# chenglou/ai-font-renderer

Hardware: AMD Instinct MI355X
Metric: glyphs/sec training (batch fwd+bwd+step) (higher is better)
Workload: dtype bf16; 1 GPU; C3: 32x32 glyph MLP 32->1024->1024->1024, char+font embedding, batch 8192/GPU (BASELINE configs[2]; per-GPU shard of configs[3]); per_gpu_batch=8192, global_batch=8192, parallelism=single, params=2137152

## Files before the change

### ai-font-renderer_amd/csrc/afr_api.hip

```cpp
#include "afr_common.h"
#include "../../include/afr.h"
static_assert(AFR_LOSS_MSE == LOSS_MSE && AFR_LOSS_BCE == LOSS_BCE, "afr.h and afr_common.h name the same loss kinds");

#include <cmath>
#include <cstdarg>
#include <cstdio>
#include <cstring>
#include <map>
#include <string>
#include <utility>
#include <vector>

static thread_local char g_err[512] = "";
static int fail(int code, const char* fmt, ...) {
    va_list ap;
    va_start(ap, fmt);
    vsnprintf(g_err, sizeof g_err, fmt, ap);
    va_end(ap);
    return code;
}
#define HIPCHK(expr)                                                                          \
    do {                                                                                      \
        hipError_t e_ = (expr);                                                               \
        if (e_ != hipSuccess) return fail(AFR_EHIP, "%s: %s", #expr, hipGetErrorString(e_)); \
// ... 39 lines not shown
    char* ws = nullptr;
    size_t ws_bytes = 0, ws_need = 0;
    int device = -1;
    bool defer = false;
    int pend_tile256 = 0;
    std::vector<GemmParams> pend;
    std::vector<std::string> pend_tag;
    double pend_flops = 0.0, pend_bytes = 0.0;
    unsigned* pend_arrived = nullptr;
    size_t o_shadow = 0, o_err = 0, o_loss = 0, o_u = 0, o_z = 0, o_dz = 0, o_slab_e = 0, o_save = 0;
    std::vector<size_t> o_act;
    size_t o_d[2] = {0, 0};
    size_t o_table = 0;
    size_t o_dw1 = 0;
    int k0 = 0;
    bool fused1 = false;
    bool wT_valid = false;
    size_t o_w1t = 0, o_w2t = 0, o_slab1 = 0;
    bool l1f = false; size_t o_l1f = 0;
    bool combo_ok = false, combo_on = false; size_t o_h1c = 0, o_h0c = 0, o_cidx = 0; int h1c_ld = 0;
    std::vector<size_t> o_mbits; bool mbits_on = false;
    size_t o_shadow2 = 0; int shadow_cur = 0;
    bool step_on = false; AdamArgs st{};
    std::vector<int64_t> adam_done;
    struct PixBlock { int64_t ln1g, ln1b, win, bin, wo, bo, ln2g, ln2b, w1, b1, w2, b2; };
    std::vector<PixBlock> pix;
    int64_t px_pos = 0, px_emb = 0, px_font = -1, px_lnfg = 0, px_lnfb = 0, px_wout = 0, px_bout = 0;
    struct PixSave { size_t hin, h1, n1, q, o, n2, kv, f, ln1p, ln2p, fbits; };
    std::vector<PixSave> pxs;
    size_t o_ctx = 0, o_a = 0, o_hf = 0, o_dh = 0, o_dht = 0, o_df = 0, o_dn = 0, o_dq = 0, o_dkvp = 0, o_dkv = 0, o_dkvt = 0, o_dctxt = 0,
           o_dctx = 0, o_headp = 0;
    struct Layer { int N, K; int64_t w_off, b_off; int sk = 1; size_t o_slab_w = 0, o_slab_b = 0;
                   size_t o_cnt = 0; int n_cnt = 0; unsigned coop_arrived = 0; };
    std::vector<Layer> layers;
    std::vector<Layer> pxl;
    int64_t emb_off = 0, font_off = 0;
    int64_t s_pos = 0, s_emb = 0, s_win = 0, s_bin = 0, s_wo = 0, s_bo = 0, s_g = 0, s_b = 0, s_w1 = 0, s_b1 = 0, s_wout = 0, s_bout = 0;
    const int64_t* last_x = nullptr;
    const int64_t* last_font = nullptr;
    int last_B = 0, last_L = 0, last_ldx = 0, last_training = 0;
    uint64_t last_step = 0;
    bool have_du = false;
    bool have_u = false;
    int next_stage = 0;
    const int64_t* ds_x = nullptr; const int64_t* ds_font = nullptr; const void* ds_target = nullptr;
    int ds_tdtype = 0, ds_L = 0; int64_t ds_rows = 0;
// ... 875 lines not shown
            h = p->ws + p->o_h1c;
            first = 1;
        } else if (p->k0) {
            const auto& l = p->layers[0];
            ProfScope ps(p, s, "glyph_l1_fwd", 0.0, (double)B * l.N * p->act_bytes);
            HIPCHK(afr_launch_glyph_l1_fwd(c.dtype, p->P + p->emb_off, femb, p->P + l.w_off, p->P + l.b_off, x, font, B, c.embed_dim,
                                           l.N, c.vocab, c.n_fonts, (float*)(p->ws + p->o_table), h, p->ws + p->o_act[1], err, s,
                                           p->l1f ? (void*)(p->ws + p->o_w1t) : nullptr));
            h = p->ws + p->o_act[1];
            first = 1;
        } else {
            ProfScope ps(p, s, "glyph_embed", 0.0, 0.0);
            HIPCHK(afr_launch_glyph_embed(c.dtype, p->P + p->emb_off, femb, x, font, B, c.embed_dim, c.vocab, c.n_fonts, h, err, s));
        }
        const bool bits = fl != nullptr && c.dtype == AFR_BF16;
        for (int i = first; i < nl; ++i) {
            const auto& l = p->layers[i];
            const bool last = (i == nl - 1);
            void* outp = last ? u : (void*)(p->ws + p->o_act[i + 1]);
            GemmParams g = lin_fwd(p, l, h, outp, B, last ? 0 : AFR_GEMM_RELU);
            if (combo && i == 1) { g.a_rowmap = (const int*)(p->ws + p->o_cidx); g.lda = p->h1c_ld; }
            if (bits && !last && p->o_mbits[i]) { g.mask_out = (unsigned char*)(p->ws + p->o_mbits[i]); g.ldmask = l.N / 8; }
            if (last && fl) g.loss = *fl;
            int rc = run_gemm(p, s, g);
            if (rc) return rc;
            h = outp;
        }
        p->last_L = 1;
    }
    if (y) {
        ProfScope ps(p, s, c.loss == AFR_LOSS_BCE ? "sigmoid_out" : "clamp_out", 0.0, 0.0);
        HIPCHK(afr_launch_clamp_out(c.dtype, u, y, (long long)B * Pix, s, c.loss));
    }
    p->last_x = x; p->last_font = font; p->last_B = B; p->last_training = training; p->last_step = step;
    p->next_stage = 0;
    p->combo_on = c.kind == AFR_KIND_GLYPH && fl != nullptr && p->k0 && combo_for(p, B);
    p->mbits_on = c.kind == AFR_KIND_GLYPH && fl != nullptr && c.dtype == AFR_BF16;
    p->have_du = fl != nullptr;
    p->have_u = fl == nullptr;
    return AFR_OK;
}
extern "C" int afr_forward(afr_plan* p, const int64_t* x, const int64_t* font, int B, int L, float* y, int training,
                           uint64_t step, void* stream) {
    return forward_impl(p, x, font, B, L, y, training, step, stream, nullptr);
}

// ... 159 lines not shown
            return AFR_OK;
        }
        if ((rc = run_gemm(p, s, lin_dx(p, p->layers[0], du, p->ws + p->o_dz, nullptr, B)))) return rc;
        if ((rc = sheet_front_bwd(p, s, rt, 7.0e6))) return rc;
        if ((rc = flush())) return rc;
        if (g_off) *g_off = 0;
        if (g_len) *g_len = p->s_wout;
        return AFR_OK;
    }
    const int nl = (int)p->layers.size();
    const int i = nl - 1 - stage;
    auto& l = p->layers[i];
    const void* a = p->ws + p->o_act[i];
    const void* dy = stage == 0 ? du : (const void*)(p->ws + p->o_d[(stage - 1) & 1]);
    if (i == 0 && p->k0) {
        const int K0 = p->k0, E = c.embed_dim;
        if (p->l1f && !(c.reserved & AFR_CFG_L1_BWD_UNFUSED)) {
            float* sl = (float*)(p->ws + p->o_l1f);
            const int CS = afr_glyph_l1_bwd_fused_split(B, l.N), nb = afr_glyph_l1_bwd_fused_blocks(B, l.N), nc = l.N / CS;
            const long long st = afr_glyph_l1_bwd_fused_slab_floats(B, l.N, c.vocab, c.n_fonts);
            {
                ProfScope ps(p, s, "glyph_l1_bwd_fused", 2.0 * B * l.N * (2.0 * E + 1.0), (double)B * l.N * 2.0 + (double)nb * st * 4.0);
                if (p->combo_on) HIPCHK(afr_launch_glyph_l1_bwd_fused(dy, l.N, p->ws + p->o_h0c, E, p->ws + p->o_w1t, p->last_x, p->last_font, B, l.N,
                                                                      c.vocab, c.n_fonts, sl, s, (const int*)(p->ws + p->o_cidx)));
                else HIPCHK(afr_launch_glyph_l1_bwd_fused(dy, l.N, a, K0, p->ws + p->o_w1t, p->last_x, p->last_font, B, l.N, c.vocab, c.n_fonts, sl, s));
            }
            for (int cs = 0; cs < CS; ++cs) {
                afr_rtable_add(rt, p->G + l.w_off + (size_t)cs * nc * E, sl + (size_t)cs * st, nb / CS, st * CS, (long long)nc * E);
                afr_rtable_add(rt, p->G + l.b_off + (size_t)cs * nc, sl + (size_t)cs * st + (size_t)nc * E, nb / CS, st * CS, nc);
            }
            afr_rtable_add(rt, p->G + p->emb_off, sl + (size_t)nc * E + nc, nb, st, (long long)c.vocab * E);
            if (c.n_fonts > 0) afr_rtable_add(rt, p->G + p->font_off, sl + (size_t)nc * E + nc + (size_t)c.vocab * E, nb, st, (long long)c.n_fonts * E);
            if ((rc = flush())) return rc;
            if (g_off) *g_off = 0;
            if (g_len) *g_len = l.b_off + (l.N + 63) / 64 * 64;
            return AFR_OK;
        }
        int sk = choose_splitk(l.N, K0, B);
        if (sk > l.sk) sk = l.sk;
        float* sw = (float*)(p->ws + l.o_slab_w);
        float* sb = (float*)(p->ws + l.o_slab_b);
        const long long stride = (long long)l.N * K0;
        if ((rc = run_gemm(p, s, lin_dw(dy, a, sw, sk == 1 ? p->G + l.b_off : sb, B, l.N, K0, sk, sk == 1 ? 0 : stride)))) return rc;
        if (sk > 1) afr_rtable_add(rt, p->G + l.b_off, sb, sk, l.N, l.N);
        float* dw1 = (float*)(p->ws + p->o_dw1);
        float* part = (float*)(p->ws + p->o_slab_e);
        {
            ProfScope ps(p, s, "glyph_l1_bwd", 0.0, (double)sk * l.N * K0 * 4.0);
// ... 390 lines not shown
                           int L, int64_t mean_elems, float* loss_accum, uint64_t step, int do_step, float lr, float b1,
                           float b2, float eps, float wd, int64_t t, void* stream) {
    int rc;
    if ((rc = check_loss_args(target, tdtype, mean_elems, loss_accum))) return rc;
    if (!p || !p->P) return fail(AFR_ESTATE, "plan has no bound parameters");
    if ((rc = ema_guard(p, "afr_train_step"))) return rc;
    DevGuard dg(p->device);
    const AdamArgs h{lr, b1, b2, eps, wd, t};
    const bool fuse_opt = do_step && !(p->cfg.reserved & AFR_CFG_UNFUSED_OPTIMIZER) && !(p->clip_norm > 0.f);
    if (p->fused1 && !(p->cfg.reserved & AFR_CFG_NO_FUSED_GLYPH1)) {
        if (!p->G) return fail(AFR_ESTATE, "plan has no bound gradient buffer");
        RTable rt;
        if ((rc = glyph1_fused(p, x, font, target, tdtype, rowmap, B, mean_elems, loss_accum, (hipStream_t)stream, rt))) return rc;
        if (fuse_opt && moments_bound(p)) {
            if (t < 1) return fail(AFR_EINVAL, "t starts at 1");
            rc = reduce_and_step(p, (hipStream_t)stream, rt, h);
            p->wT_valid = rc == AFR_OK;
            return rc;
        }
        if ((rc = run_reduce_group(p, (hipStream_t)stream, rt))) return rc;
        if (do_step && (rc = afr_adamw_step(p, lr, b1, b2, eps, wd, t, 1.f, stream))) return rc;
        return AFR_OK;
    }
    const LossArgs fl = loss_args(p, true, target, tdtype, rowmap, mean_elems, loss_accum);
    if ((rc = forward_impl(p, x, font, B, L, nullptr, 1, step, stream, &fl))) return rc;
    if (fuse_opt && fused_step_eligible(p, B)) {
        if (t < 1) return fail(AFR_EINVAL, "t starts at 1");
        return sheet_fused_step(p, (hipStream_t)stream, h);
    }
    if (fuse_opt && moments_bound(p) && p->cfg.kind != AFR_KIND_PIXEL) {
        if (t < 1) return fail(AFR_EINVAL, "t starts at 1");
        const int n = afr_backward_stages(p);
        RTable rt;
        p->step_on = true; p->adam_done.clear(); p->st = h;
        for (int st = 0; st < n; ++st)
            if ((rc = backward_stage_impl(p, st, nullptr, nullptr, (hipStream_t)stream, &rt))) { p->step_on = false; return rc; }
        p->step_on = false;
        p->next_stage = 0;
        p->have_du = false;
        return reduce_and_step(p, (hipStream_t)stream, rt, h);
    }
    if ((rc = afr_backward(p, stream))) return rc;
    if (do_step && (rc = afr_adamw_step(p, lr, b1, b2, eps, wd, t, 1.f, stream))) return rc;
    return AFR_OK;
}
extern "C" int afr_train_step(afr_plan* p, const int64_t* x, const int64_t* font, const void* target, int tdtype, int B,
                              int L, int64_t mean_elems, float* loss_accum, uint64_t step, int do_step, float lr, float b1,
                              float b2, float eps, float wd, int64_t t, void* stream) {
    return train_step_impl(p, x, font, target, tdtype, nullptr, B, L, mean_elems, loss_accum, step, do_step, lr, b1, b2, eps, wd, t, stream);
}

extern "C" int afr_bind_dataset(afr_plan* p, const int64_t* x, const int64_t* font, const void* target, int tdtype, int64_t n_rows, int L) {
    if (!p) return fail(AFR_EINVAL, "null plan");
    if (!x && !font && !target) {
        p->ds_x = p->ds_font = nullptr; p->ds_target = nullptr; p->ds_rows = 0; p->ds_L = 0;
        return AFR_OK;
    }
    if (n_rows >= (1ll << 31)) return fail(AFR_EUNSUPPORTED, "a data set of %lld rows: row indices are narrowed to 32 bits (fewer than 2^31 rows)", (long long)n_rows);
    if (!x || !target || n_rows <= 0) return fail(AFR_EINVAL, "a data set needs codes, targets and at least one row");
// ... 455 lines not shown
```

### ai-font-renderer_amd/csrc/afr_common.h

```cpp
#pragma once
#include <hip/hip_runtime.h>
#include <stdint.h>
#include <stddef.h>
#include <type_traits>

typedef __bf16 bf16_t;
typedef __attribute__((ext_vector_type(4))) float f32x4;
typedef __attribute__((ext_vector_type(16))) float f32x16;
typedef __attribute__((ext_vector_type(8))) __bf16 bf16x8;
typedef __attribute__((ext_vector_type(4))) __bf16 bf16x4;
typedef __attribute__((ext_vector_type(4))) short s16x4;

__host__ __device__ __forceinline__ uint32_t afr_hash32(uint64_t idx, uint32_t key) {
    uint32_t lo = (uint32_t)idx, hi = (uint32_t)(idx >> 32);
    uint32_t h = lo * 0x9E3779B1u + (key + hi * 0x85EBCA6Bu);
    h ^= h >> 16; h *= 0x21F0AAADu;
    h ^= h >> 15; h *= 0x735A2D97u;
    h ^= h >> 15;
    return h;
}
__host__ __device__ __forceinline__ bool afr_keep(uint64_t idx, uint32_t key, uint32_t thr24) {
    return (afr_hash32(idx, key) >> 8) < thr24;
}

// ... 1 lines not shown
    uint64_t z = x + 0x9E3779B97F4A7C15ull;
    z = (z ^ (z >> 30)) * 0xBF58476D1CE4E5B9ull;
    z = (z ^ (z >> 27)) * 0x94D049BB133111EBull;
    return z ^ (z >> 31);
}
enum { AFR_STREAM_EMBED = 1, AFR_STREAM_ATTN = 2, AFR_STREAM_FC = 3 };
static inline uint32_t afr_dropout_key(uint64_t seed, uint64_t step, uint64_t stream, uint64_t rank) {
    uint64_t v = seed ^ (step * 0x9E3779B97F4A7C15ull) ^ (stream * 0xC2B2AE3D27D4EB4Full) ^ (rank * 0x165667B19E3779F9ull);
    return (uint32_t)(afr_splitmix64(v) & 0xFFFFFFFFull);
}
static inline uint32_t afr_keep_threshold(float keep_prob) { return (uint32_t)((double)keep_prob * 16777216.0); }

__device__ __forceinline__ float wave_sum(float v) {
#pragma unroll
    for (int o = 32; o > 0; o >>= 1) v += __shfl_xor(v, o, 64);
    return v;
}
__device__ __forceinline__ float wave_max(float v) {
#pragma unroll
    for (int o = 32; o > 0; o >>= 1) v = fmaxf(v, __shfl_xor(v, o, 64));
    return v;
}

__device__ __forceinline__ void loss_block_finish(float block_sum, float* partial, unsigned* counter, float* loss_accum,
                                                  float inv_n, float* sh) {
    __shared__ unsigned ticket_;
    if (threadIdx.x == 0) {
        __hip_atomic_store(partial + blockIdx.x, block_sum, __ATOMIC_RELAXED, __HIP_MEMORY_SCOPE_AGENT);
        asm volatile("s_waitcnt vmcnt(0)" ::: "memory");
        ticket_ = __hip_atomic_fetch_add(counter, 1u, __ATOMIC_RELAXED, __HIP_MEMORY_SCOPE_AGENT);
    }
    __syncthreads();
    if (ticket_ != gridDim.x - 1) return;
    float a = 0.f;
    for (int i = threadIdx.x; i < (int)gridDim.x; i += blockDim.x)
        a += __hip_atomic_load(partial + i, __ATOMIC_RELAXED, __HIP_MEMORY_SCOPE_AGENT);
    sh[threadIdx.x] = a;
    __syncthreads();
    for (int o = blockDim.x >> 1; o > 0; o >>= 1) {
        if ((int)threadIdx.x < o) sh[threadIdx.x] += sh[threadIdx.x + o];
        __syncthreads();
    }
    if (threadIdx.x == 0) {
        loss_accum[0] += sh[0] * inv_n;
        __hip_atomic_store(counter, 0u, __ATOMIC_RELAXED, __HIP_MEMORY_SCOPE_AGENT);
    }
}

constexpr int LOSS_MSE = 0, LOSS_BCE = 1;
__device__ __forceinline__ float sigmoid_of(float u, float e) {
    const float r = __builtin_amdgcn_rcpf(1.f + e);
    return u >= 0.f ? r : e * r;
}
__device__ __forceinline__ float sigmoid_f(float u) { return sigmoid_of(u, __expf(-fabsf(u))); }
__device__ __forceinline__ float bce_logits_elem(float u, float t, float inv_n, float& du) {
    const float e = __expf(-fabsf(u));
    du = (sigmoid_of(u, e) - t) * inv_n;
    return fmaf(-t, u, fmaxf(u, 0.f)) + __logf(1.f + e);
}
template <int LOSS>
__device__ __forceinline__ float loss_elem(float u, float t, float inv_n, float g2, float& du) {
    if constexpr (LOSS == LOSS_BCE) return bce_logits_elem(u, t, inv_n, du);
    else {
        const float diff = fminf(fmaxf(u, 0.f), 1.f) - t;
        du = (u >= 0.f && u <= 1.f) ? g2 * diff : 0.f;
        return diff * diff;
    }
}
template <bool LUT>
// ... 73 lines not shown
    int M, N, K;
    int lda, ldb, ldc, ldaux;
    int flags;
    int splitk;
    long long slab_stride;
    float* colsum = nullptr;
    long long colsum_stride = 0;
    LossArgs loss;
    float* ad_p = nullptr; float* ad_m = nullptr; float* ad_v = nullptr; bf16_t* ad_shadow = nullptr;
    AdamHyper ad;
    int head_tiles = 0;
    int ad_kind = OPT_ADAMW;
    float* fix_ws = nullptr; unsigned* fix_cnt = nullptr;
    float* coop_ws = nullptr; unsigned* coop_cnt = nullptr; unsigned coop_target = 0; uint32_t* err = nullptr;
    const int* a_rowmap = nullptr; const int* b_rowmap = nullptr; const int* aux_rowmap = nullptr;
    float out_scale = 1.f;
    unsigned char* mask_out = nullptr; const unsigned char* mask_in = nullptr; int ldmask = 0;
#ifdef AFR_GEMM_TIMING
    int dbg_slot = 0;
#endif
};
constexpr uint32_t AFR_ERR_INDEX = 1u, AFR_ERR_COOP_TIMEOUT = 2u, AFR_ERR_ROW = 4u, AFR_ERR_GRAD_NONFINITE = 8u;
hipError_t afr_launch_gemm(int dtype, const GemmParams& p, hipStream_t s);
hipError_t afr_launch_gemm_fp8(const GemmParams& p, hipStream_t s);
hipError_t afr_launch_f32_to_fp8(const float* src, unsigned char* dst, long long n, float inv_scale, hipStream_t s);
bool afr_gemm_groupable(int dtype, const GemmParams& p);
hipError_t afr_launch_gemm_group(int dtype, const GemmParams* ps, int n, int tile256, hipStream_t s);
void afr_gemm_pair_plan(int B, int n_out, int k_in, int* tile256, int* splitk);
constexpr size_t AFR_FIX_SLICE_BYTES = 256 * 256 * 4;
hipError_t afr_launch_gemm_fix(const GemmParams& p, hipStream_t s);
const char* afr_gemm_kernel_name(int dtype, const GemmParams& p);
bool afr_gemm_wide_ok(int M, int N, int K);

hipError_t afr_launch_reduce(float* dst, const float* slabs, int nslabs, long long slab_stride, long long n,
                             float scale, int accumulate, hipStream_t s);
struct RSeg {
    float* dst; const float* src; long long stride; long long n4; int nslabs; int blk0; int nblk; int deep;
    bf16_t* shT = nullptr; int tN = 0, tK = 0;
};
constexpr int AFR_RT_MAXSEG = 32;
constexpr int AFR_L1F_MAX_SPLIT = 4;
struct RTable {
    int nseg = 0; int nblocks = 0; int overflow = 0;
    int adam = 0; AdamHyper ad;
    const float* gbase; float* P; float* M; float* V; bf16_t* shadow;
    RSeg seg[AFR_RT_MAXSEG];
// ... 35 lines not shown
                                   int* ridx, int64_t* sx, int64_t* sfont, uint32_t* err_flag, hipStream_t s);
hipError_t afr_launch_f32_to_bf16(const float* src, bf16_t* dst, long long n, hipStream_t s);
hipError_t afr_launch_clamp_bwd(int act_dtype, void* u_inout, const float* dy, long long n, hipStream_t s, int loss_kind = LOSS_MSE);
hipError_t afr_launch_clamp_out(int act_dtype, const void* u, float* y, long long n, hipStream_t s, int loss_kind = LOSS_MSE);
hipError_t afr_launch_glyph_embed(int act_dtype, const float* emb, const float* font_emb, const int64_t* x,
                                  const int64_t* font, int B, int E, int vocab, int n_fonts, void* out,
                                  uint32_t* err_flag, hipStream_t s);
int afr_embed_bwd_blocks(int B);
hipError_t afr_launch_glyph_l1_fwd(int act_dtype, const float* emb, const float* font_emb, const float* W1, const float* b1,
                                   const int64_t* x, const int64_t* font, int B, int E, int N1, int vocab, int n_fonts,
                                   float* table, void* h0, void* h1, uint32_t* err_flag, hipStream_t s, void* w1t = nullptr);
hipError_t afr_launch_glyph_combo(const float* emb, const float* font_emb, const float* W1, const float* b1, const int64_t* x,
                                  const int64_t* font, int B, int E, int N1, int vocab, int n_fonts, float* table, void* h1c,
                                  int ld1 , void* h0c, int* cidx, uint32_t* err_flag, hipStream_t s,
                                  void* w1t);
int afr_glyph_k0(int E, int vocab, int n_fonts);
int afr_glyph_l1_bwd_blocks(int N1);
bool afr_glyph_l1_bwd_fused_eligible(int dtype, int E, int N1, int vocab, int n_fonts);
int afr_glyph_l1_bwd_fused_split(int B, int N1);
int afr_glyph_l1_bwd_fused_blocks(int B, int N1);
long long afr_glyph_l1_bwd_fused_slab_floats(int B, int N1, int vocab, int n_fonts);
hipError_t afr_launch_glyph_l1_bwd_fused(const void* d1, int ldd, const void* h0, int ldh, const void* W1T, const int64_t* x,
                                         const int64_t* font, int B, int N1, int vocab, int n_fonts, float* slabs, hipStream_t s,
                                         const int* h0_rowmap = nullptr);
hipError_t afr_launch_glyph_l1_bwd(const float* slabs, int nslabs, long long slab_stride, const float* W1, int N1, int E,
                                   int vocab, int n_fonts, float* dw1, float* dtab_part, hipStream_t s);
hipError_t afr_launch_glyph_embed_bwd(int act_dtype, const void* d, const int64_t* x, const int64_t* font, int B,
                                      int E, int vocab, int n_fonts, float* slabs ,
                                      hipStream_t s);

struct SheetDims { int L, Lmax, E, H, F, vocab; };
constexpr int AFR_SHEET_SAVE_PER_POS = 56;
struct SheetParams {
    const float *pos, *emb, *w_in, *b_in, *w_o, *b_o, *ln_g, *ln_b, *w1, *b1;
};
struct SheetDrop {
    uint32_t key_e, key_a, key_f, thr_e, thr_a, thr_f; float sc_e, sc_a, sc_f; int training;
    float* save;
    float* dbg_e0 = nullptr;
};
struct SheetSlabOff { int pos, emb, win, bin, wo, bo, g, b, w1, b1, total; };
extern "C" int afr_sheet_blocks(int B);
size_t afr_sheet_fwd_lds_bytes(const SheetDims& d);
size_t afr_sheet_bwd_lds_bytes(const SheetDims& d);
hipError_t afr_launch_sheet_fwd(int act_dtype, const SheetDims& d, const SheetParams& P, const SheetDrop& dr,
                                const int64_t* x, int ldx, int B, void* z, float ln_eps, uint32_t* err_flag,
                                hipStream_t s);
// ... 44 lines not shown
```

### ai-font-renderer_amd/csrc/gemm.hip

```cpp
#include <cstdlib>
#include "afr_common.h"
#include "../../include/afr.h"

__device__ __forceinline__ int xcd_walk(int b, int nb) {
    const int q = nb >> 3, r = nb & 7, xcd = b & 7, idx = b >> 3;
    return (xcd < r ? xcd * (q + 1) : r * (q + 1) + (xcd - r) * q) + idx;
}
__device__ __forceinline__ void tile_coords(const GemmParams& p, int BM, int BN, int t, int q, int r, int& tm, int& tn) {
    const int tiles_m = (p.M + BM - 1) / BM, tiles_n = (p.N + BN - 1) / BN;
    const int tiles = tiles_m * tiles_n;
    const bool n_slow = p.N > p.M;
    const int ts = n_slow ? tiles_n : tiles_m, tf = n_slow ? tiles_m : tiles_n;
    int G = 8;
    if (r == 0 && q % tf == 0 && q / tf >= 1 && q / tf < 8 && tiles % q == 0) G = q / tf;
    const int grp = t / (G * tf);
    const int s0 = grp * G;
    const int gs = min(G, ts - s0);
    const int rr = t - grp * G * tf;
    const bool fast_first = tf <= 8;
    const int sidx = fast_first ? s0 + rr / tf : s0 + rr % gs, fidx = fast_first ? rr % tf : rr / gs;
    tm = n_slow ? fidx : sidx;
    tn = n_slow ? sidx : fidx;
}
__device__ __forceinline__ void tile_of_block(const GemmParams& p, int BM, int BN, int b, int nb, int& tm, int& tn, int& z) {
// ... 946 lines not shown
            p.colsum[(size_t)z * p.colsum_stride + m0 + tid] = a;
        }
        __syncthreads();
    }
    const bool mse = p.loss.target != nullptr;
    float lsum = 0.f;
    const float* lut255 = nullptr;
    if (WM == 4 && mse && p.loss.tdtype == AFR_TARGET_U8) {
        float* l = reinterpret_cast<float*>(smem) + NW * 4096;
        if (tid < 256) l[tid] = (float)tid / 255.0f;
        __syncthreads();
        lut255 = l;
    }
    wave_epilogue<ALAY, BLAY, WM, false, true, TROWS, LOSS, OPT>(p, acc, m0 + wm * 64, n0 + wn * 64, z, reinterpret_cast<float*>(smem) + wave * 4096, lane, lsum, lut255);
    if (mse) {
        float* red = reinterpret_cast<float*>(smem);
        __syncthreads();
        lsum = wave_sum(lsum);
        if (lane == 0) red[wave] = lsum;
        __syncthreads();
        float bs = 0.f;
#pragma unroll
        for (int w = 0; w < NW; ++w) bs += red[w];
        loss_block_finish(bs, p.loss.partial, p.loss.counter, p.loss.loss_accum, p.loss.inv_n, red + 16);
    }
#ifdef AFR_GEMM_TIMING
    asm volatile("s_waitcnt vmcnt(0)" ::: "memory");
    __syncthreads();
    GSTAMP(3);
#endif
}

template <int ALAY, int BLAY, int GB = 0, int OPT = OPT_ADAMW>
__device__ __forceinline__ void gemm_bf16_256_body(const GemmParams& p, const int bid, const int nblk, char* smem) {
    static_assert(!GB || BLAY == 1, "row gather: k-strided B on the 256x256 kernel");
    constexpr int BM = 256, BNN = 256;
    const int tid = threadIdx.x, lane = tid & 63;
    const int wave = __builtin_amdgcn_readfirstlane(tid >> 6);
    const int wr = wave >> 2, wc = wave & 3;
    int tm, tn, z, ksplit = p.splitk;
    int tail_idx = -1;
    if (p.fix_ws) {
        const int tiles = ((p.M + BM - 1) / BM) * ((p.N + BNN - 1) / BNN);
        const int head = min(p.head_tiles, tiles), ntail = tiles - head;
        int t;
        if (bid < head) { t = xcd_walk(bid, head); z = 0; ksplit = 1; }
        else {
// ... 182 lines not shown
        float* red = reinterpret_cast<float*>(smem);
        const int c = tid % CH, rg = tid / CH;
#pragma unroll
        for (int r = 0; r < 8; ++r) red[rg * BM + 8 * c + r] = cs8[r];
        __syncthreads();
        if (tid < BM && m0 + tid < p.M) {
            float a = 0.f;
#pragma unroll
            for (int g = 0; g < 16; ++g) a += red[g * BM + tid];
            p.colsum[(size_t)z * p.colsum_stride + m0 + tid] = a;
        }
        __syncthreads();
    }
    if ((ALAY == 1 && BLAY == 1) && p.coop_ws) {
        const int S = p.splitk, per = 8 / S;
        const int T = tm * ((p.N + BNN - 1) / BNN) + tn;
        const __amdgpu_buffer_rsrc_t rws = __builtin_amdgcn_make_buffer_rsrc(p.coop_ws, 0, 0x7FFFFFFF, 0x00020000);
        typedef __attribute__((ext_vector_type(4))) unsigned u32x4;
        const unsigned tile_b = (unsigned)T * (unsigned)S * (8u * 32u * 1024u);
        float* Wt = reinterpret_cast<float*>(smem) + wave * 4096;
        {
            const unsigned mine = tile_b + ((unsigned)z * 8u + (unsigned)wave) * (32u * 1024u) + (unsigned)lane * 16u;
#pragma unroll
            for (int i = 0; i < 8; ++i)
#pragma unroll
                for (int j = 0; j < 4; ++j)
                    __builtin_amdgcn_raw_buffer_store_b128(__builtin_bit_cast(u32x4, acc[i][j]), rws, mine + (unsigned)(i * 4 + j) * 1024u, 0, 16);
        }
        asm volatile("s_waitcnt vmcnt(0)" ::: "memory");
        __syncthreads();
        GSTAMP(6);
        if (wave == 0) {
            if (lane == 0) (void)__hip_atomic_fetch_add(p.coop_cnt + T, 1u, __ATOMIC_RELAXED, __HIP_MEMORY_SCOPE_AGENT);
            unsigned spins = 0;
            while ((int)(__hip_atomic_load(p.coop_cnt + T, __ATOMIC_RELAXED, __HIP_MEMORY_SCOPE_AGENT) - p.coop_target) < 0) {
                __builtin_amdgcn_s_sleep(8);
                if (++spins > (1u << 22)) {
                    if (lane == 0 && p.err) atomicOr(p.err, AFR_ERR_COOP_TIMEOUT);
                    break;
                }
            }
        }
        __syncthreads();
        GSTAMP(7);
        for (int ii = 0; ii < per; ++ii) {
            const int i = z * per + ii;
            const unsigned src = tile_b + (unsigned)wave * (32u * 1024u) + (unsigned)(i * 4) * 1024u + (unsigned)lane * 16u;
            f32x4 v[4];
#pragma unroll
            for (int j = 0; j < 4; ++j) v[j] = (f32x4){0.f, 0.f, 0.f, 0.f};
#pragma unroll
            for (int h = 0; h < 2; ++h) {
                f32x4 q[4][4];
#pragma unroll
                for (int zq = 0; zq < 4; ++zq) {
                    const int zz = 4 * h + zq;
                    const unsigned vo = zz < S ? src + (unsigned)zz * (8u * 32u * 1024u) : 0x80000000u;
#pragma unroll
                    for (int j = 0; j < 4; ++j)
                        q[zq][j] = __builtin_bit_cast(f32x4, __builtin_amdgcn_raw_buffer_load_b128(rws, vo, (unsigned)j * 1024u, 16));
                }
#pragma unroll
                for (int j = 0; j < 4; ++j)
#pragma unroll
                    for (int zq = 0; zq < 4; ++zq) v[j] += q[zq][j];
            }
            strip_finish<OPT>(p, v, m0 + wr * 128 + 16 * i, n0 + wc * 64, Wt, lane, false);
        }
#ifdef AFR_GEMM_TIMING
        asm volatile("s_waitcnt vmcnt(0)" ::: "memory");
        __syncthreads();
        GSTAMP(3);
#endif
        return;
    }
    if (tail_idx >= 0) {
        f32x4* ws = reinterpret_cast<f32x4*>(p.fix_ws) + ((size_t)tail_idx * p.splitk * 8 + wave) * 2048 + lane;
        {
            f32x4* mine = ws + (size_t)z * 8 * 2048;
#pragma unroll
            for (int i = 0; i < 8; ++i)
#pragma unroll
                for (int j = 0; j < 4; ++j) mine[(i * 4 + j) * 64] = acc[i][j];
        }
        __threadfence();
        __syncthreads();
        unsigned* flag = reinterpret_cast<unsigned*>(smem);
        if (tid == 0) *flag = atomicAdd(p.fix_cnt + tail_idx, 1u);
// ... 64 lines not shown
    group_member(g, [&](const GemmParams& p, int bid, int nblk, auto a, auto b) {
        if constexpr (a() && b()) {
            if (p.b_rowmap) { gemm_bf16_256_body<1, 1, 1>(p, bid, nblk, smem); return; }
        }
        gemm_bf16_256_body<a(), b()>(p, bid, nblk, smem);
    });
}
__global__ __launch_bounds__(512, 2) void gemm_bf16_group256_lion(GemmGroup g) {
    __shared__ __attribute__((aligned(16))) char smem[10 * SUB];
    group_member(g, [&](const GemmParams& p, int bid, int nblk, auto a, auto b) {
        if constexpr (a() && b()) {
            if (p.b_rowmap) gemm_bf16_256_body<1, 1, 1, OPT_LION>(p, bid, nblk, smem);
            else gemm_bf16_256_body<1, 1, 0, OPT_LION>(p, bid, nblk, smem);
        } else gemm_bf16_256_body<a(), b()>(p, bid, nblk, smem);
    });
}

struct L1BwdArgs {
    const bf16_t* d1; const bf16_t* h0; const bf16_t* W1T; const int64_t* x; const int64_t* font;
    const int* h0_rowmap;
    int ldd, ldh, B, N1, vocab, n_fonts;
    int CS, ncols;
    float* slabs; long long slab_stride; int o_b, o_tab;
};
constexpr int L1_E = 32, L1_R = 64, L1_LDR = L1_R + 8;
__global__ __launch_bounds__(512) void glyph_l1_bwd_fused_kernel(L1BwdArgs a) {
    extern __shared__ __attribute__((aligned(16))) char sm[];
    const int tid = threadIdx.x, lane = tid & 63, wave = __builtin_amdgcn_readfirstlane(tid >> 6), r = lane & 15, q = lane >> 4;
    const int NS = a.ncols >> 7;
    const int rb = blockIdx.x / a.CS, n_lo = (blockIdx.x - rb * a.CS) * a.ncols;
    const int b0 = rb * L1_R, nb = min(L1_R, a.B - b0);
    char* Dimg = sm;
    char* Himg = sm + NS * SUB;
    int* ids = reinterpret_cast<int*>(sm + (NS + 1) * SUB);
    const unsigned lds0 = (unsigned)(size_t)(__attribute__((address_space(3))) char*)sm;
    float* slab = a.slabs + (size_t)blockIdx.x * a.slab_stride;
    constexpr int L1_MAXKS = 32;
    bf16x8 wv[L1_MAXKS];
    {
        const int erow = (wave & 1) * 16 + r;
        const bf16_t* wrow = a.W1T + (size_t)erow * a.N1 + n_lo + 8 * q;
        const int nks = a.ncols >> 5;
#pragma unroll
        for (int j = 0; j < L1_MAXKS; ++j)
            if (j < nks) wv[j] = *reinterpret_cast<const bf16x8*>(wrow + j * 32);
    }
    {
        const i32x4 rD = make_rsrc(a.d1), rH = make_rsrc(a.h0);
        const int pieces = (NS + 1) * 16;
        for (int pc = wave; pc < pieces; pc += 8) {
// ... 299 lines not shown
    for (int i = 0; i < n; ++i) {
        const bool kk = (ps[i].flags & AFR_GEMM_A_KSTRIDED) && (ps[i].flags & AFR_GEMM_B_KSTRIDED);
        if (ps[i].a_rowmap || (ps[i].b_rowmap && !(ok && n > 1 && tile256 && kk)) || (ps[i].aux_rowmap && !(ps[i].flags & AFR_GEMM_OUT_BF16)))
            return hipErrorInvalidValue;
    }
    for (int i = 0; i < n; ++i) {
        if (!ps[i].coop_ws) continue;
        const long long tiles = (long long)((ps[i].M + 255) / 256) * ((ps[i].N + 255) / 256);
        const int S = ps[i].splitk;
        if (i != 0 || !ok || !tile256 || !ps[i].coop_cnt || (S != 2 && S != 4 && S != 8) || tiles * S > 256 ||
            tiles * S * (long long)AFR_FIX_SLICE_BYTES >= (1ll << 31)) return hipErrorInvalidValue;
        coop = true;
    }
    if (!ok || (n == 1 && !coop)) {
        for (int i = 0; i < n; ++i) { hipError_t e = afr_launch_gemm(dtype, ps[i], s); if (e != hipSuccess) return e; }
        return hipSuccess;
    }
#ifdef AFR_GEMM_TIMING
    GemmParams q[4];
    { const int slot = g_dbg_slot++ & 63; for (int i = 0; i < n; ++i) { q[i] = ps[i]; q[i].dbg_slot = slot; } }
    ps = q;
#endif
    return launch_grouped(ps, n, tile256, true, s);
}
hipError_t afr_launch_gemm(int dtype, const GemmParams& p_in, hipStream_t s) {
#ifdef AFR_GEMM_TIMING
    GemmParams p = p_in;
    DBG_SLOT(p);
#else
    const GemmParams& p = p_in;
#endif
    const int a = (p.flags & AFR_GEMM_A_KSTRIDED) ? 1 : 0, b = (p.flags & AFR_GEMM_B_KSTRIDED) ? 1 : 0;
    if (p.M <= 0 || p.N <= 0) return hipSuccess;
    if (p.loss.kind != LOSS_MSE && p.loss.kind != LOSS_BCE) return hipErrorInvalidValue;
    const bool bce = p.loss.kind == LOSS_BCE && p.loss.target, trows = p.loss.rowmap != nullptr;
    if (bce && (a || b || p.a_rowmap || p.splitk != 1)) return hipErrorInvalidValue;
    if (trows && (!p.loss.target || a || b || p.a_rowmap || p.splitk != 1 || (dtype == AFR_BF16 && bf16_use_body256(p)))) return hipErrorInvalidValue;
    if (p.a_rowmap || p.b_rowmap || p.aux_rowmap) {
        if (dtype != AFR_BF16 || p.b_rowmap || (p.a_rowmap && (a || b || !bf16_use_wide(p))) ||
            (p.aux_rowmap && !(p.flags & AFR_GEMM_OUT_BF16))) return hipErrorInvalidValue;
    }
    if (dtype == AFR_BF16 && bf16_use_body256(p)) return launch_grouped(&p, 1, true, false, s);
    const bool wide = dtype == AFR_BF16 && bf16_use_wide(p);
    const int tiles = ((p.M + (wide ? 255 : 127)) / (wide ? 256 : 128)) * ((p.N + 127) / 128);
    auto launch = [&](auto kernel, int threads) { hipLaunchKernelGGL(kernel, dim3(tiles * p.splitk), dim3(threads), 0, s, p); };
    auto variant = [&](auto al, auto bl, auto tr, auto loss) {
        if (dtype == AFR_BF16) {
            if (wide) launch(bf16k::gemm_bf16<al(), bl(), 4, 0, tr(), loss()>, 512);
            else launch(bf16k::gemm_bf16<al(), bl(), 2, 0, tr(), loss()>, 256);
        } else if (dtype == AFR_BF16X3) launch(x3k::gemm_bf16x3<al(), bl(), tr(), loss()>, 256);
        else launch(f32k::gemm_f32<al(), bl(), tr(), loss()>, 256);
    };
    if (p.ad_p && p.ad_kind == OPT_LION) {
        if (!a || !b || p.loss.target || p.a_rowmap || wide) return hipErrorInvalidValue;
        constexpr int MSE = LOSS_MSE;
        if (dtype == AFR_BF16) launch(bf16k::gemm_bf16<1, 1, 2, 0, false, MSE, OPT_LION>, 256);
        else if (dtype == AFR_BF16X3) launch(x3k::gemm_bf16x3<1, 1, false, MSE, OPT_LION>, 256);
        else launch(f32k::gemm_f32<1, 1, false, MSE, OPT_LION>, 256);
    } else if (p.ad_p && p.ad_kind != OPT_ADAMW) return hipErrorInvalidValue;
    else if (p.a_rowmap) launch(bf16k::gemm_bf16<0, 0, 4, 1>, 512);
    else if (bce || trows)
        with_bool(trows, [&](auto tr) { with_loss(bce ? LOSS_BCE : LOSS_MSE, [&](auto loss) { variant(std::false_type{}, std::false_type{}, tr, loss); }); });
    else
        with_bool(a, [&](auto al) { with_bool(b, [&](auto bl) { variant(al, bl, std::false_type{}, std::integral_constant<int, LOSS_MSE>{}); }); });
    return hipGetLastError();
}

bool afr_glyph_l1_bwd_fused_eligible(int dtype, int E, int N1, int vocab, int n_fonts) {
    return dtype == AFR_BF16 && E == bf16k::L1_E && N1 % 128 == 0 && N1 >= 256 && N1 <= 1024 && vocab + n_fonts <= 144;
}
int afr_glyph_l1_bwd_fused_split(int B, int N1) {
    const int nrb = (B + bf16k::L1_R - 1) / bf16k::L1_R;
    int cs = 1;
    while (cs * 2 <= AFR_L1F_MAX_SPLIT && cs * 2 * nrb <= 256 && N1 % (cs * 2 * 128) == 0) cs *= 2;
    return cs;
}
int afr_glyph_l1_bwd_fused_blocks(int B, int N1) { return (B + bf16k::L1_R - 1) / bf16k::L1_R * afr_glyph_l1_bwd_fused_split(B, N1); }
long long afr_glyph_l1_bwd_fused_slab_floats(int B, int N1, int vocab, int n_fonts) {
    const int nc = N1 / afr_glyph_l1_bwd_fused_split(B, N1);
    return (long long)nc * bf16k::L1_E + nc + (long long)(vocab + n_fonts) * bf16k::L1_E;
}
hipError_t afr_launch_glyph_l1_bwd_fused(const void* d1, int ldd, const void* h0, int ldh, const void* W1T, const int64_t* x,
                                         const int64_t* font, int B, int N1, int vocab, int n_fonts, float* slabs, hipStream_t s,
                                         const int* h0_rowmap) {
    if (B <= 0) return hipSuccess;
    bf16k::L1BwdArgs a;
    a.d1 = (const bf16_t*)d1; a.h0 = (const bf16_t*)h0; a.W1T = (const bf16_t*)W1T; a.x = x; a.font = font; a.h0_rowmap = h0_rowmap;
    a.ldd = ldd; a.ldh = ldh; a.B = B; a.N1 = N1; a.vocab = vocab; a.n_fonts = n_fonts;
    a.CS = afr_glyph_l1_bwd_fused_split(B, N1); a.ncols = N1 / a.CS;
    a.slabs = slabs; a.slab_stride = afr_glyph_l1_bwd_fused_slab_floats(B, N1, vocab, n_fonts);
    a.o_b = a.ncols * bf16k::L1_E; a.o_tab = a.o_b + a.ncols;
    const size_t lds = (size_t)(a.ncols / 128 + 1) * bf16k::SUB + 2 * bf16k::L1_R * sizeof(int);
    static size_t set[16];
    int dev = 0;
    if (lds > 48 * 1024 && hipGetDevice(&dev) == hipSuccess && (dev < 0 || dev >= 16 || set[dev] < lds)) {
        hipError_t e = hipFuncSetAttribute((const void*)bf16k::glyph_l1_bwd_fused_kernel, hipFuncAttributeMaxDynamicSharedMemorySize, (int)lds);
        if (e != hipSuccess) return e;
        if (dev >= 0 && dev < 16) set[dev] = lds;
    }
    hipLaunchKernelGGL(bf16k::glyph_l1_bwd_fused_kernel, dim3(afr_glyph_l1_bwd_fused_blocks(B, N1)), dim3(512), lds, s, a);
    return hipGetLastError();
}
```

Measured before the change: 44.50 million glyphs/s.

## Defer loss reduction to extra block of L1 backward kernel; skip self split-K reload

The last forward GEMM no longer runs the atomic ticket and last-block loss reduction. It only writes per-block partial sums, and the final sum is done by one extra block appended to the fused layer-1 backward kernel. This removes a serialising atomic counter and a waitcnt from the GEMM epilogue. Separately, the split-K reduction in the grouped GEMM keeps each wave's own slice in registers instead of storing it and reloading it, which cuts LDS or workspace traffic. The risks are extra register pressure from the select chain, and the loss is only valid once backward has run.

```diff
diff --git a/ai-font-renderer_amd/csrc/afr_api.hip b/ai-font-renderer_amd/csrc/afr_api.hip
--- a/ai-font-renderer_amd/csrc/afr_api.hip
+++ b/ai-font-renderer_amd/csrc/afr_api.hip
@@ -85,6 +85,7 @@
     std::vector<size_t> o_mbits; bool mbits_on = false;
     size_t o_shadow2 = 0; int shadow_cur = 0;
     bool step_on = false; AdamArgs st{};
+    LossSum loss_defer{};
     std::vector<int64_t> adam_done;
     struct PixBlock { int64_t ln1g, ln1b, win, bin, wo, bo, ln2g, ln2b, w1, b1, w2, b2; };
     std::vector<PixBlock> pix;
@@ -1006,6 +1007,10 @@
             if (combo && i == 1) { g.a_rowmap = (const int*)(p->ws + p->o_cidx); g.lda = p->h1c_ld; }
             if (bits && !last && p->o_mbits[i]) { g.mask_out = (unsigned char*)(p->ws + p->o_mbits[i]); g.ldmask = l.N / 8; }
             if (last && fl) g.loss = *fl;
+            if (last && fl && !fl->counter) {
+                p->loss_defer.partial = fl->partial; p->loss_defer.inv_n = fl->inv_n; p->loss_defer.loss_accum = fl->loss_accum;
+                afr_gemm_tile_launch_shape(p->gemm_dtype, g, &p->loss_defer.n, &p->loss_defer.bd);
+            }
             int rc = run_gemm(p, s, g);
             if (rc) return rc;
             h = outp;
@@ -1211,8 +1216,10 @@
             {
                 ProfScope ps(p, s, "glyph_l1_bwd_fused", 2.0 * B * l.N * (2.0 * E + 1.0), (double)B * l.N * 2.0 + (double)nb * st * 4.0);
                 if (p->combo_on) HIPCHK(afr_launch_glyph_l1_bwd_fused(dy, l.N, p->ws + p->o_h0c, E, p->ws + p->o_w1t, p->last_x, p->last_font, B, l.N,
-                                                                      c.vocab, c.n_fonts, sl, s, (const int*)(p->ws + p->o_cidx)));
-                else HIPCHK(afr_launch_glyph_l1_bwd_fused(dy, l.N, a, K0, p->ws + p->o_w1t, p->last_x, p->last_font, B, l.N, c.vocab, c.n_fonts, sl, s));
+                                                                      c.vocab, c.n_fonts, sl, s, (const int*)(p->ws + p->o_cidx), &p->loss_defer));
+                else HIPCHK(afr_launch_glyph_l1_bwd_fused(dy, l.N, a, K0, p->ws + p->o_w1t, p->last_x, p->last_font, B, l.N, c.vocab, c.n_fonts, sl, s,
+                                                          nullptr, &p->loss_defer));
+                p->loss_defer = LossSum{};
             }
             for (int cs = 0; cs < CS; ++cs) {
                 afr_rtable_add(rt, p->G + l.w_off + (size_t)cs * nc * E, sl + (size_t)cs * st, nb / CS, st * CS, (long long)nc * E);
@@ -1649,8 +1656,12 @@
         if (do_step && (rc = afr_adamw_step(p, lr, b1, b2, eps, wd, t, 1.f, stream))) return rc;
         return AFR_OK;
     }
-    const LossArgs fl = loss_args(p, true, target, tdtype, rowmap, mean_elems, loss_accum);
-    if ((rc = forward_impl(p, x, font, B, L, nullptr, 1, step, stream, &fl))) return rc;
+    LossArgs fl = loss_args(p, true, target, tdtype, rowmap, mean_elems, loss_accum);
+    p->loss_defer = LossSum{};
+    const bool defer_loss = fuse_opt && t >= 1 && !fused_step_eligible(p, B) && moments_bound(p) && p->cfg.kind == AFR_KIND_GLYPH && p->k0 &&
+                            p->l1f && !(p->cfg.reserved & AFR_CFG_L1_BWD_UNFUSED) && p->gemm_dtype == AFR_BF16;
+    if (defer_loss) fl.counter = nullptr;
+    if ((rc = forward_impl(p, x, font, B, L, nullptr, 1, step, stream, &fl))) { p->loss_defer = LossSum{}; return rc; }
     if (fuse_opt && fused_step_eligible(p, B)) {
         if (t < 1) return fail(AFR_EINVAL, "t starts at 1");
         return sheet_fused_step(p, (hipStream_t)stream, h);
@@ -1661,7 +1672,7 @@
         RTable rt;
         p->step_on = true; p->adam_done.clear(); p->st = h;
         for (int st = 0; st < n; ++st)
-            if ((rc = backward_stage_impl(p, st, nullptr, nullptr, (hipStream_t)stream, &rt))) { p->step_on = false; return rc; }
+            if ((rc = backward_stage_impl(p, st, nullptr, nullptr, (hipStream_t)stream, &rt))) { p->step_on = false; p->loss_defer = LossSum{}; return rc; }
         p->step_on = false;
         p->next_stage = 0;
         p->have_du = false;
diff --git a/ai-font-renderer_amd/csrc/afr_common.h b/ai-font-renderer_amd/csrc/afr_common.h
--- a/ai-font-renderer_amd/csrc/afr_common.h
+++ b/ai-font-renderer_amd/csrc/afr_common.h
@@ -47,9 +47,14 @@
     return v;
 }
 
+template <bool DEFERRABLE = false>
 __device__ __forceinline__ void loss_block_finish(float block_sum, float* partial, unsigned* counter, float* loss_accum,
                                                   float inv_n, float* sh) {
     __shared__ unsigned ticket_;
+    if (DEFERRABLE && !counter) {
+        if (threadIdx.x == 0) __hip_atomic_store(partial + blockIdx.x, block_sum, __ATOMIC_RELAXED, __HIP_MEMORY_SCOPE_AGENT);
+        return;
+    }
     if (threadIdx.x == 0) {
         __hip_atomic_store(partial + blockIdx.x, block_sum, __ATOMIC_RELAXED, __HIP_MEMORY_SCOPE_AGENT);
         asm volatile("s_waitcnt vmcnt(0)" ::: "memory");
@@ -70,6 +75,26 @@
         loss_accum[0] += sh[0] * inv_n;
         __hip_atomic_store(counter, 0u, __ATOMIC_RELAXED, __HIP_MEMORY_SCOPE_AGENT);
     }
+}
+struct LossSum {
+    const float* partial = nullptr;
+    int n = 0, bd = 0;
+    float inv_n = 0.f;
+    float* loss_accum = nullptr;
+};
+__device__ __forceinline__ void loss_sum_deferred(const LossSum& l, float* sh) {
+    const int t = threadIdx.x, bd = l.bd;
+    if (t < bd) {
+        float a = 0.f;
+        for (int i = t; i < l.n; i += bd) a += l.partial[i];
+        sh[t] = a;
+    }
+    __syncthreads();
+    for (int o = bd >> 1; o > 0; o >>= 1) {
+        if (t < o) sh[t] += sh[t + o];
+        __syncthreads();
+    }
+    if (t == 0) l.loss_accum[0] += sh[0] * l.inv_n;
 }
 
 constexpr int LOSS_MSE = 0, LOSS_BCE = 1;
@@ -189,6 +214,7 @@
 };
 constexpr uint32_t AFR_ERR_INDEX = 1u, AFR_ERR_COOP_TIMEOUT = 2u, AFR_ERR_ROW = 4u, AFR_ERR_GRAD_NONFINITE = 8u;
 hipError_t afr_launch_gemm(int dtype, const GemmParams& p, hipStream_t s);
+void afr_gemm_tile_launch_shape(int dtype, const GemmParams& p, int* tiles, int* threads);
 hipError_t afr_launch_gemm_fp8(const GemmParams& p, hipStream_t s);
 hipError_t afr_launch_f32_to_fp8(const float* src, unsigned char* dst, long long n, float inv_scale, hipStream_t s);
 bool afr_gemm_groupable(int dtype, const GemmParams& p);
@@ -270,7 +296,7 @@
 long long afr_glyph_l1_bwd_fused_slab_floats(int B, int N1, int vocab, int n_fonts);
 hipError_t afr_launch_glyph_l1_bwd_fused(const void* d1, int ldd, const void* h0, int ldh, const void* W1T, const int64_t* x,
                                          const int64_t* font, int B, int N1, int vocab, int n_fonts, float* slabs, hipStream_t s,
-                                         const int* h0_rowmap = nullptr);
+                                         const int* h0_rowmap = nullptr, const LossSum* loss = nullptr);
 hipError_t afr_launch_glyph_l1_bwd(const float* slabs, int nslabs, long long slab_stride, const float* W1, int N1, int E,
                                    int vocab, int n_fonts, float* dw1, float* dtab_part, hipStream_t s);
 hipError_t afr_launch_glyph_embed_bwd(int act_dtype, const void* d, const int64_t* x, const int64_t* font, int B,
diff --git a/ai-font-renderer_amd/csrc/gemm.hip b/ai-font-renderer_amd/csrc/gemm.hip
--- a/ai-font-renderer_amd/csrc/gemm.hip
+++ b/ai-font-renderer_amd/csrc/gemm.hip
@@ -992,7 +992,7 @@
         float bs = 0.f;
 #pragma unroll
         for (int w = 0; w < NW; ++w) bs += red[w];
-        loss_block_finish(bs, p.loss.partial, p.loss.counter, p.loss.loss_accum, p.loss.inv_n, red + 16);
+        loss_block_finish<true>(bs, p.loss.partial, p.loss.counter, p.loss.loss_accum, p.loss.inv_n, red + 16);
     }
 #ifdef AFR_GEMM_TIMING
     asm volatile("s_waitcnt vmcnt(0)" ::: "memory");
@@ -1221,10 +1221,12 @@
         {
             const unsigned mine = tile_b + ((unsigned)z * 8u + (unsigned)wave) * (32u * 1024u) + (unsigned)lane * 16u;
 #pragma unroll
-            for (int i = 0; i < 8; ++i)
+            for (int i = 0; i < 8; ++i) {
+                if ((unsigned)(i - z * per) < (unsigned)per) continue;
 #pragma unroll
                 for (int j = 0; j < 4; ++j)
                     __builtin_amdgcn_raw_buffer_store_b128(__builtin_bit_cast(u32x4, acc[i][j]), rws, mine + (unsigned)(i * 4 + j) * 1024u, 0, 16);
+            }
         }
         asm volatile("s_waitcnt vmcnt(0)" ::: "memory");
         __syncthreads();
@@ -1245,6 +1247,13 @@
         for (int ii = 0; ii < per; ++ii) {
             const int i = z * per + ii;
             const unsigned src = tile_b + (unsigned)wave * (32u * 1024u) + (unsigned)(i * 4) * 1024u + (unsigned)lane * 16u;
+            f32x4 own[4];
+#pragma unroll
+            for (int j = 0; j < 4; ++j) {
+                own[j] = acc[0][j];
+#pragma unroll
+                for (int i2 = 1; i2 < 8; ++i2) own[j] = i == i2 ? acc[i2][j] : own[j];
+            }
             f32x4 v[4];
 #pragma unroll
             for (int j = 0; j < 4; ++j) v[j] = (f32x4){0.f, 0.f, 0.f, 0.f};
@@ -1254,7 +1263,7 @@
 #pragma unroll
                 for (int zq = 0; zq < 4; ++zq) {
                     const int zz = 4 * h + zq;
-                    const unsigned vo = zz < S ? src + (unsigned)zz * (8u * 32u * 1024u) : 0x80000000u;
+                    const unsigned vo = (zz < S && zz != z) ? src + (unsigned)zz * (8u * 32u * 1024u) : 0x80000000u;
 #pragma unroll
                     for (int j = 0; j < 4; ++j)
                         q[zq][j] = __builtin_bit_cast(f32x4, __builtin_amdgcn_raw_buffer_load_b128(rws, vo, (unsigned)j * 1024u, 16));
@@ -1262,7 +1271,7 @@
 #pragma unroll
                 for (int j = 0; j < 4; ++j)
 #pragma unroll
-                    for (int zq = 0; zq < 4; ++zq) v[j] += q[zq][j];
+                    for (int zq = 0; zq < 4; ++zq) v[j] += (4 * h + zq == z) ? own[j] : q[zq][j];
             }
             strip_finish<OPT>(p, v, m0 + wr * 128 + 16 * i, n0 + wc * 64, Wt, lane, false);
         }
@@ -1373,10 +1382,16 @@
     int ldd, ldh, B, N1, vocab, n_fonts;
     int CS, ncols;
     float* slabs; long long slab_stride; int o_b, o_tab;
+    int nwork;
+    LossSum loss;
 };
 constexpr int L1_E = 32, L1_R = 64, L1_LDR = L1_R + 8;
 __global__ __launch_bounds__(512) void glyph_l1_bwd_fused_kernel(L1BwdArgs a) {
     extern __shared__ __attribute__((aligned(16))) char sm[];
+    if ((int)blockIdx.x >= a.nwork) {
+        loss_sum_deferred(a.loss, reinterpret_cast<float*>(sm));
+        return;
+    }
     const int tid = threadIdx.x, lane = tid & 63, wave = __builtin_amdgcn_readfirstlane(tid >> 6), r = lane & 15, q = lane >> 4;
     const int NS = a.ncols >> 7;
     const int rb = blockIdx.x / a.CS, n_lo = (blockIdx.x - rb * a.CS) * a.ncols;
@@ -1722,6 +1737,11 @@
     ps = q;
 #endif
     return launch_grouped(ps, n, tile256, true, s);
+}
+void afr_gemm_tile_launch_shape(int dtype, const GemmParams& p, int* tiles, int* threads) {
+    const bool wide = dtype == AFR_BF16 && bf16_use_wide(p);
+    *tiles = ((p.M + (wide ? 255 : 127)) / (wide ? 256 : 128)) * ((p.N + 127) / 128);
+    *threads = wide ? 512 : 256;
 }
 hipError_t afr_launch_gemm(int dtype, const GemmParams& p_in, hipStream_t s) {
 #ifdef AFR_GEMM_TIMING
@@ -1742,7 +1762,8 @@
     }
     if (dtype == AFR_BF16 && bf16_use_body256(p)) return launch_grouped(&p, 1, true, false, s);
     const bool wide = dtype == AFR_BF16 && bf16_use_wide(p);
-    const int tiles = ((p.M + (wide ? 255 : 127)) / (wide ? 256 : 128)) * ((p.N + 127) / 128);
+    int tiles, threads_;
+    afr_gemm_tile_launch_shape(dtype, p, &tiles, &threads_);
     auto launch = [&](auto kernel, int threads) { hipLaunchKernelGGL(kernel, dim3(tiles * p.splitk), dim3(threads), 0, s, p); };
     auto variant = [&](auto al, auto bl, auto tr, auto loss) {
         if (dtype == AFR_BF16) {
@@ -1782,8 +1803,9 @@
 }
 hipError_t afr_launch_glyph_l1_bwd_fused(const void* d1, int ldd, const void* h0, int ldh, const void* W1T, const int64_t* x,
                                          const int64_t* font, int B, int N1, int vocab, int n_fonts, float* slabs, hipStream_t s,
-                                         const int* h0_rowmap) {
+                                         const int* h0_rowmap, const LossSum* loss) {
     if (B <= 0) return hipSuccess;
+    if (loss && loss->partial && (loss->n < 1 || (loss->bd != 256 && loss->bd != 512) || !loss->loss_accum)) return hipErrorInvalidValue;
     bf16k::L1BwdArgs a;
     a.d1 = (const bf16_t*)d1; a.h0 = (const bf16_t*)h0; a.W1T = (const bf16_t*)W1T; a.x = x; a.font = font; a.h0_rowmap = h0_rowmap;
     a.ldd = ldd; a.ldh = ldh; a.B = B; a.N1 = N1; a.vocab = vocab; a.n_fonts = n_fonts;
@@ -1798,6 +1820,8 @@
         if (e != hipSuccess) return e;
         if (dev >= 0 && dev < 16) set[dev] = lds;
     }
-    hipLaunchKernelGGL(bf16k::glyph_l1_bwd_fused_kernel, dim3(afr_glyph_l1_bwd_fused_blocks(B, N1)), dim3(512), lds, s, a);
+    a.nwork = afr_glyph_l1_bwd_fused_blocks(B, N1);
+    if (loss && loss->partial) a.loss = *loss;
+    hipLaunchKernelGGL(bf16k::glyph_l1_bwd_fused_kernel, dim3(a.nwork + (a.loss.partial ? 1 : 0)), dim3(512), lds, s, a);
     return hipGetLastError();
 }
```

After: 45.42 million glyphs/s (median of 6 runs). 1.02x the previous value.
